# KIT-MBS/pydca

Hardware: AMD Instinct MI355X
Metric: plmDCA L-BFGS iterations/s (L=500 N=50000 q=21) (higher is better)
Workload: dtype f32

## Files before the change

### include/dca_hip.h

```cpp
#ifndef DCA_HIP_H
#define DCA_HIP_H

#include <stdbool.h>
#include <stddef.h>
#include <stdint.h>

#ifdef __cplusplus
extern "C" {
#endif

#define DCA_OK 0
#define DCA_ERR_ARG (-1)
#define DCA_ERR_IO (-2)
#define DCA_ERR_RESIDUE (-3)
#define DCA_ERR_NOMEM (-4)
#define DCA_ERR_HIP (-5)
#define DCA_ERR_NO_DEVICE (-6)
#define DCA_ERR_NOT_SPD (-7)
#define DCA_ERR_STATE (-8)

#define DCA_BIOMOLECULE_PROTEIN 1
#define DCA_BIOMOLECULE_RNA 2

#define DCA_F32 32
// ... 80 lines not shown
typedef int (*dca_comm_hook)(void* user, int op, void* buf_dev, size_t count, int dtype);
int dca_plm_set_vector_sharding(dca_ctx* ctx, int rank, int world, dca_comm_hook hook, void* user);

typedef struct {
    int status;
    int iterations;
    int evaluations;
    int finished;
    double fx, xnorm, gnorm, step;
    double seconds;
} dca_plm_stats;

int dca_plm_lbfgs_begin(dca_ctx* ctx, int max_iterations, int verbose);
int dca_plm_lbfgs_iterate(dca_ctx* ctx, int iterations, dca_plm_stats* stats_out);
int dca_plm_lbfgs_end(dca_ctx* ctx);

typedef struct dca_plm_args {
    int biomolecule;
    const char* msa_file;
    const uint8_t* msa;
    int num_seqs, seqs_len;
    float seqid, lambda_h, lambda_J;
    int max_iterations;
    int precision;
    const int* devices;
    int num_devices;
    int exchange_scheme;
    const char* rccl_path;
    int verbose;
} dca_plm_args;
// ... 130 lines not shown
```

### pydca_amd/_lib.py

```python
import ctypes as C
import os
import subprocess

import numpy as np

_HERE = os.path.dirname(os.path.abspath(__file__))
LIB_PATH = os.environ.get("DCA_LIB_PATH") or os.path.join(_HERE, "lib", "libdca_hip.so")

DCA_OK = 0
DCA_ERR_ARG, DCA_ERR_IO, DCA_ERR_RESIDUE = -1, -2, -3
DCA_ERR_NOMEM, DCA_ERR_HIP, DCA_ERR_NO_DEVICE, DCA_ERR_NOT_SPD, DCA_ERR_STATE = -4, -5, -6, -7, -8
DCA_F32, DCA_F64 = 32, 64
DCA_BIOMOLECULE_PROTEIN, DCA_BIOMOLECULE_RNA = 1, 2
CARRY_EXACT, CARRY_CHUNKED, CARRY_SERIAL = 0, 1, 2
PROTEIN, RNA = 1, 2


class DcaBackendError(RuntimeError):
    def __init__(self, code, msg):
        super().__init__("libdca_hip error %d: %s" % (code, msg))
        self.code = code


class PlmStats(C.Structure):
    _fields_ = [("status", C.c_int), ("iterations", C.c_int), ("evaluations", C.c_int), ("finished", C.c_int),
                ("fx", C.c_double), ("xnorm", C.c_double), ("gnorm", C.c_double), ("step", C.c_double),
                ("seconds", C.c_double)]
# ... 80 lines not shown
        "dca_plm_num_params": (sz, [i, i]),
        "dca_plm_init_x": (i, [vp]),
        "dca_plm_set_x": (i, [vp, vp, i]),
        "dca_plm_get_x": (i, [vp, vp, i]),
        "dca_plm_release": (i, [vp]),
        "dca_plm_gradient": (i, [vp, C.POINTER(d)]),
        "dca_plm_get_g": (i, [vp, vp, i]),
        "dca_plm_set_reduce_hook": (i, [vp, REDUCE_HOOK, vp]),
        "dca_mf_set_reduce_hook": (i, [vp, REDUCE_HOOK, vp]),
        "dca_di_from_arrays": (i, [vp, vp, i, vp, i, i, vp, vp]),
        "dca_di_from_fields": (i, [vp, vp, i, vp, vp, i, i, vp]),
        "dca_plm_set_vector_sharding": (i, [vp, i, i, COMM_HOOK, vp]),
        "dca_plm_lbfgs_begin": (i, [vp, i, i]),
        "dca_plm_lbfgs_iterate": (i, [vp, i, C.POINTER(PlmStats)]),
        "dca_plm_lbfgs_end": (i, [vp]),
        "dca_mf_set_row_window": (i, [vp, i, i]),
        "dca_comm_allgather_host": (i, [vp, vp, i, vp]),
        "dca_plm_scores": (i, [vp, i, vp]),
        "dca_plm_di_scores": (i, [vp, vp, i, vp]),
        "dca_mf_di_scores": (i, [vp, i, vp]),
        "dca_plm_pair_couplings": (i, [vp, vp, i, i, vp]),
        "dca_mf_fields": (i, [vp, vp]),
        "dca_encode_sequences": (i, [C.c_char_p, vp, i, i, i, i, vp, C.POINTER(i)]),
        "dca_plm_energies": (i, [vp, vp, i, vp]),
        "dca_plm_mutation_scan": (i, [vp, vp, vp]),
        "dca_mf_energies": (i, [vp, vp, i, vp]),
        "dca_mf_mutation_scan": (i, [vp, vp, vp]),
        "dca_plm_pseudo_likelihood": (i, [vp, vp, i, vp, vp, vp]),
        "dca_mf_pseudo_likelihood": (i, [vp, vp, i, vp, vp, vp]),
        "dca_plm_sample": (i, [vp, i, i, C.c_uint64, C.c_uint64, C.c_uint64, d, vp, vp]),
# ... 52 lines not shown
    }
    for name, (res, args) in sig.items():
        f = getattr(L, name)
        f.restype = res
        f.argtypes = args
    _lib = L
    return L


EXPORTS = ["dca_weights_work", "dca_compute_weights_sharded", "dca_weights_partial_counts", "dca_set_weight_counts", "dca_comm_unique_id",
           "dca_comm_init", "dca_comm_destroy", "dca_comm_abort", "dca_comm_info", "dca_plm_set_native_comm", "dca_mf_set_native_comm",
           "dca_last_error", "dca_version", "dca_device_count", "dca_release_cached_memory", "dca_device_blocks_in_use", "dca_read_msa", "dca_count_msa_lines", "dca_read_msa_alloc", "dca_mf_set_row_window", "dca_comm_allgather_host", "dca_fasta_shape", "dca_read_fasta", "dca_read_fasta_alloc", "dca_host_free", "dca_create",
           "dca_destroy", "dca_set_msa", "dca_compute_weights", "dca_set_weights", "dca_get_weights",
           "dca_get_weight_counts", "dca_get_meff", "dca_plm_configure", "dca_plm_configure_strips", "dca_plm_num_params", "dca_plm_init_x",
           "dca_plm_set_x", "dca_plm_get_x", "dca_plm_release", "dca_plm_gradient", "dca_plm_get_g", "dca_plm_set_reduce_hook", "dca_mf_set_reduce_hook", "dca_di_from_arrays", "dca_di_from_fields", "dca_plm_set_vector_sharding",
           "dca_plm_lbfgs_begin", "dca_plm_lbfgs_iterate", "dca_plm_lbfgs_end", "dca_plm_scores", "dca_plm_di_scores",
           "dca_mf_di_scores", "dca_plm_pair_couplings", "dca_mf_fields", "dca_mf_pair_couplings",
           "dca_encode_sequences", "dca_plm_energies", "dca_plm_mutation_scan", "dca_mf_energies", "dca_mf_mutation_scan",
           "dca_plm_pseudo_likelihood", "dca_mf_pseudo_likelihood",
           "dca_plm_sample", "dca_mf_sample", "dca_philox4x32_10",
           "dca_ar_configure", "dca_ar_num_params", "dca_ar_init_x", "dca_ar_set_x", "dca_ar_get_x", "dca_ar_gradient", "dca_ar_get_g",
           "dca_ar_fit", "dca_ar_log_probabilities", "dca_ar_sample", "dca_ar_release",
           "dca_ar_epistasis", "dca_ar_epistatic_scores",
           "dca_plm_bm_begin", "dca_plm_bm_iterate", "dca_plm_bm_freqs", "dca_plm_bm_chains", "dca_plm_bm_end",
           "dca_plm_ais", "dca_mf_ais", "dca_ais_estimate",
           "dca_hamming_nearest", "dca_sequence_statistics", "dca_alignment_statistics",
           "dca_three_site_values", "dca_three_site_scan", "dca_pca_fit", "dca_pca_project",
           "dca_mf_single_site_freqs",
           "dca_mf_pair_site_freqs", "dca_mf_corr_mat", "dca_mf_couplings", "dca_mf_scores", "dca_mf_run",
           "dca_mf_corr_from_freqs", "dca_spd_inverse", "dca_sw_scores", "dca_sw_align", "dca_scores_order", "dca_set_profiling", "dca_set_profiling_only", "dca_get_kernel_time",
           "dca_reset_kernel_times", "dca_plm_run", "plmdcaBackend", "freeFieldsAndCouplings"]
# ... 378 lines not shown
                return 1
        self._mf_hook = REDUCE_HOOK(tramp) if pyfunc is not None else C.cast(None, REDUCE_HOOK)
        check(self._l.dca_mf_set_reduce_hook(self._h, self._mf_hook, None))

    def plm_lbfgs_begin(self, max_iterations, verbose=False):
        check(self._l.dca_plm_lbfgs_begin(self._h, int(max_iterations), int(bool(verbose))))

    def plm_lbfgs_end(self):
        check(self._l.dca_plm_lbfgs_end(self._h))

    def plm_lbfgs_iterate(self, iterations):
        st = PlmStats()
        check(self._l.dca_plm_lbfgs_iterate(self._h, int(iterations), C.byref(st)))
        return st

    def plm_scores(self, apc=True):
        out = np.zeros(self.L * (self.L - 1) // 2, dtype=np.float64)
        check(self._l.dca_plm_scores(self._h, int(bool(apc)), _ptr(out)))
        return out

    def plm_di_scores(self, reg_fi, apc=False):
        reg_fi = np.ascontiguousarray(reg_fi, dtype=np.float64)
        if reg_fi.shape != (self.L, self.q):
            raise ValueError("reg_fi must be L x q")
        out = np.zeros(self.L * (self.L - 1) // 2, dtype=np.float64)
        check(self._l.dca_plm_di_scores(self._h, _ptr(reg_fi), int(bool(apc)), _ptr(out)))
        return out

    def di_from_arrays(self, couplings, layout, reg_fi, L, q, want_fields=False, want_di=True):
        couplings = np.ascontiguousarray(couplings, dtype=np.float64)
# ... 392 lines not shown
```

### pydca_amd/csrc/capi.cpp

```cpp
#include <cstdlib>

#include "dca_internal.h"

static thread_local char g_err[1024] = "";

void dca_set_error(const char* fmt, ...)
{
    va_list ap;
    va_start(ap, fmt);
    vsnprintf(g_err, sizeof(g_err), fmt, ap);
    va_end(ap);
}

void dca_flush_clocks(dca_ctx* ctx)
{
    for (auto& kv : ctx->clocks) {
        for (auto& pr : kv.second.pending) {
            float ms = 0.f;
            hipEventSynchronize(pr.second);
            if (hipEventElapsedTime(&ms, pr.first, pr.second) == hipSuccess) kv.second.ms += ms;
            hipEventDestroy(pr.first);
            hipEventDestroy(pr.second);
        }
        kv.second.pending.clear();
// ... 460 lines not shown
    if (hook && ctx->plm->native_mode == 4) { dca_set_error("configured for column strips: no reduce hook"); return DCA_ERR_STATE; }
    ctx->plm->hook = hook;
    ctx->plm->hook_user = user;
    if (hook && ctx->plm->native_mode == 1) ctx->plm->native_mode = 0;
    return DCA_OK;
}
int dca_plm_lbfgs_begin(dca_ctx* ctx, int max_iterations, int verbose)
{
    CHECK_CTX(ctx);
    DCA_TRY(need_plm(ctx));
    dca_bm_free(ctx);
    return ctx->plm->lbfgs_begin(max_iterations, verbose);
}
int dca_plm_lbfgs_iterate(dca_ctx* ctx, int iterations, dca_plm_stats* st) { CHECK_CTX(ctx); DCA_TRY(need_plm(ctx)); return ctx->plm->lbfgs_iterate(iterations, st); }
int dca_plm_lbfgs_end(dca_ctx* ctx) { CHECK_CTX(ctx); if (ctx->plm) ctx->plm->lbfgs_end(); return DCA_OK; }
int dca_plm_scores(dca_ctx* ctx, int apc, double* out) { CHECK_CTX(ctx); DCA_TRY(need_plm(ctx)); return ctx->plm->scores(apc, out); }
int dca_plm_energies(dca_ctx* ctx, const uint8_t* X, int n, double* energies_out)
{
    CHECK_CTX(ctx);
    DCA_TRY(need_plm(ctx));
    if (n < 0 || (n > 0 && (!X || !energies_out))) return DCA_ERR_ARG;
    PottsSource ps;
    DCA_TRY(ctx->plm->potts_source(&ps, false));
    return dca_potts_energies(ctx, ps, X, n, energies_out);
}
int dca_plm_mutation_scan(dca_ctx* ctx, const uint8_t* wildtype, double* dE_out)
{
    CHECK_CTX(ctx);
    DCA_TRY(need_plm(ctx));
    if (!wildtype || !dE_out) return DCA_ERR_ARG;
// ... 417 lines not shown
```

### pydca_amd/csrc/dca_internal.h

```cpp
#pragma once
#include <hip/hip_runtime.h>

#include <atomic>
#include <cstdarg>
#include <cstdint>
#include <cstdio>
#include <cstring>
#include <map>
#include <string>
#include <vector>

#include "../../include/dca_hip.h"
#include "potts_source.h"

void dca_set_error(const char* fmt, ...);

#define HIP_TRY(expr)                                                                   \
    do {                                                                                \
        hipError_t _e = (expr);                                                         \
        if (_e != hipSuccess) {                                                         \
            dca_set_error("%s failed: %s (%s:%d)", #expr, hipGetErrorString(_e), __FILE__, __LINE__); \
            return DCA_ERR_HIP;                                                         \
        }                                                                               \
    } while (0)
// ... 141 lines not shown
int dca_comm_native_sum_u32(dca_ctx* ctx, uint32_t* buf, size_t count);

struct PlmEngineBase {
    virtual ~PlmEngineBase() {}
    virtual int configure(double lambda_h, double lambda_J, int carry_mode, int chunk, int warmup,
                          int halo, int add_reg) = 0;
    virtual int configure_strips(double lambda_h, double lambda_J, int carry_mode, int chunk, int warmup) = 0;
    virtual int init_x() = 0;
    virtual int set_x(const void* x, int dtype) = 0;
    virtual int get_x(void* x, int dtype) = 0;
    virtual int get_g(void* g, int dtype) = 0;
    virtual int gradient(double* fx_out) = 0;
    virtual int lbfgs_begin(int max_iterations, int verbose) = 0;
    virtual int lbfgs_iterate(int iterations, dca_plm_stats* st) = 0;
    virtual void lbfgs_end() = 0;
    virtual int scores(int apc, double* out) = 0;
    virtual int di_scores(const double* reg_fi, int apc, double* out) = 0;
    virtual int pair_couplings(const int* pairs, int npairs, int shift, double* out) = 0;
    virtual int potts_source(PottsSource* out, bool one_gpu_only) = 0;
    virtual int bm_source(void** dx) = 0;
    virtual int set_vector_sharding(int rank, int world, dca_comm_hook hook, void* user) = 0;
    dca_reduce_hook hook = nullptr;
    void* hook_user = nullptr;
    virtual void weights_changed() = 0;
    virtual int set_native_comm(int mode) = 0;
    virtual bool configured_for_comm() const = 0;
    int native_mode = 0;
};
PlmEngineBase* dca_make_plm_engine(dca_ctx* ctx);

// ... 111 lines not shown
```

### pydca_amd/csrc/lbfgs_kernels.h

```cpp
#pragma once

#include "dca_internal.h"
#include "plm_plan.h"
#include "vec_kernels.h"

namespace {

template <bool DD> struct DotAcc;
template <> struct DotAcc<false> {
    double hi = 0.0;
    static constexpr double lo = 0.0;
    __device__ __forceinline__ void add(double a, double b) { hi += a * b; }
    __device__ __forceinline__ void wave_reduce() { for (int off = 32; off > 0; off >>= 1) hi += __shfl_down(hi, off); }
};
template <> struct DotAcc<true> {
    double hi = 0.0, lo = 0.0;
    __device__ __forceinline__ void add(double a, double b) { dd_add(hi, lo, __dmul_rn(a, b)); }
    __device__ __forceinline__ void wave_reduce() { dd_wave_reduce(hi, lo); }
};
template <int NV>
__device__ __forceinline__ void dot_block_store(double (*red)[2 * NV], int nv, double* __restrict__ partials, unsigned grid = 0)
{
    __syncthreads();
    if ((int)threadIdx.x < nv) {
// ... 19 lines not shown
            s0.add(av, bv); s1.add(cv, cv); s2.add(av, av);
        },
        { const double av = a[i]; const double bv = b[i]; const double cv = c[i]; s0.add(av, bv); s1.add(cv, cv); s2.add(av, av); })
    s0.wave_reduce(); s1.wave_reduce(); s2.wave_reduce();
    if ((threadIdx.x & 63) == 0) {
        double* r = red[threadIdx.x >> 6];
        r[0] = s0.hi; r[1] = s0.lo; r[2] = s1.hi; r[3] = s1.lo; r[4] = s2.hi; r[5] = s2.lo;
    }
    dot_block_store<3>(red, 3, partials);
}
struct VecPtrs5 { const void* s[5]; const void* y[5]; };
struct DirCoefs { double g; double s[5]; double y[5]; };

struct LbfgsDev { double SY[5][5]; double YY[5][5]; double ys[5]; DirCoefs cf; };
constexpr int kSlotDginit = 30;

__global__ void lbfgs_two_loop_kernel(double* __restrict__ scal, LbfgsDev* __restrict__ st, int e, int endNext, int bound, double gg)
{
    if (threadIdx.x != 0 || blockIdx.x != 0) return;
    constexpr int M = 5;
    const double ys = scal[1], yy = scal[2];
    const double* G5 = scal + 3;
    double Sg[M], Yg[M], alpha[M];
    st->ys[e] = ys;
    for (int k2 = 0; k2 < M; ++k2) {
        Sg[k2] = G5[k2]; Yg[k2] = G5[5 + k2];
        st->SY[e][k2] = G5[10 + k2];
        st->SY[k2][e] = G5[15 + k2];
        st->YY[e][k2] = G5[20 + k2];
        st->YY[k2][e] = G5[20 + k2];
// ... 231 lines not shown
    for (int b = lo_ + threadIdx.x; b < hi_; b += blockDim.x) dd_add2(hi, lo, parts[2 * (size_t)b], parts[2 * (size_t)b + 1]);
    dd_block_reduce(hi, lo, redHi, redLo);
    if (threadIdx.x == 0) { out[2 * blockIdx.x] = hi; out[2 * blockIdx.x + 1] = lo; }
}
__global__ __launch_bounds__(1024)
void dd_sum_final_kernel(const double* __restrict__ A, int nA, const double* __restrict__ B, int nB, double* __restrict__ out)
{
    __shared__ double redHi[1024], redLo[1024];
    double hi = 0.0, lo = 0.0;
    for (int b = threadIdx.x; b < nA; b += blockDim.x) dd_add2(hi, lo, A[2 * (size_t)b], A[2 * (size_t)b + 1]);
    for (int b = threadIdx.x; b < nB; b += blockDim.x) dd_add2(hi, lo, B[2 * (size_t)b], B[2 * (size_t)b + 1]);
    dd_block_reduce(hi, lo, redHi, redLo);
    if (threadIdx.x == 0) out[0] = hi + lo;
}

template <typename T>
__global__ __launch_bounds__(kVecThreads)
void vec_dot3_fx_kernel(const T* __restrict__ a, const T* __restrict__ b, const T* __restrict__ c, size_t n, double* __restrict__ partials,
                        const double* __restrict__ fxParts, int nFxParts, double* __restrict__ fxChunks)
{
    if (blockIdx.x >= (unsigned)kVecBlocks) {
        __shared__ double redHi[256], redLo[256];
        const int blk = (int)blockIdx.x - kVecBlocks;
        const int chunk = (nFxParts + kSumStageBlocks - 1) / kSumStageBlocks;
        const int lo_ = blk * chunk, hi_ = min(nFxParts, lo_ + chunk);
        double hi = 0.0, lo = 0.0;
        for (int p = lo_ + threadIdx.x; p < hi_; p += blockDim.x) dd_add2(hi, lo, fxParts[2 * (size_t)p], fxParts[2 * (size_t)p + 1]);
        dd_block_reduce(hi, lo, redHi, redLo);
        if (threadIdx.x == 0) { fxChunks[2 * blk] = hi; fxChunks[2 * blk + 1] = lo; }
        return;
    }
    __shared__ double red[kVecThreads / 64][6];
    DotAcc<sizeof(T) == 8> s0, s1, s2;
    DCA_VEC_LOOP_G(n, a, kVecBlocks,
        const Pack<T> pa = ldp_at(a + head_, iv); const Pack<T> pb = ldp_at(b + head_, iv); const Pack<T> pc = ldp_at(c + head_, iv);
        _Pragma("unroll") for (int k = 0; k < VEC; ++k) {
            const double av = pa.v[k]; const double bv = pb.v[k]; const double cv = pc.v[k];
            s0.add(av, bv); s1.add(cv, cv); s2.add(av, av);
        },
        { const double av = a[i]; const double bv = b[i]; const double cv = c[i]; s0.add(av, bv); s1.add(cv, cv); s2.add(av, av); })
    s0.wave_reduce(); s1.wave_reduce(); s2.wave_reduce();
    if ((threadIdx.x & 63) == 0) {
        double* r = red[threadIdx.x >> 6];
        r[0] = s0.hi; r[1] = s0.lo; r[2] = s1.hi; r[3] = s1.lo; r[4] = s2.hi; r[5] = s2.lo;
    }
    dot_block_store<3>(red, 3, partials, kVecBlocks);
}
__global__ __launch_bounds__(1024)
void vec_final_fx_kernel(const double* __restrict__ partials, int nb, int nk, double* __restrict__ out,
                         const double* __restrict__ A, int nA, const double* __restrict__ B, int nB, double* __restrict__ fxOut)
{
    __shared__ double redHi[1024], redLo[1024];
    const int k = blockIdx.x;
    double hi = 0.0, lo = 0.0;
    if (k < nk) {
        constexpr int NT = 256;
        if ((int)threadIdx.x < NT) {
            for (int b = threadIdx.x; b < nb; b += NT) dd_add2(hi, lo, partials[2 * ((size_t)k * nb + b)], partials[2 * ((size_t)k * nb + b) + 1]);
            redHi[threadIdx.x] = hi;
            redLo[threadIdx.x] = lo;
        }
        __syncthreads();
        for (int st = NT / 2; st > 0; st >>= 1) {
            if ((int)threadIdx.x < st) dd_add2(redHi[threadIdx.x], redLo[threadIdx.x], redHi[threadIdx.x + st], redLo[threadIdx.x + st]);
            __syncthreads();
        }
        if (threadIdx.x == 0) out[k] = redHi[0] + redLo[0];
        return;
    }
    for (int b = threadIdx.x; b < nA; b += blockDim.x) dd_add2(hi, lo, A[2 * (size_t)b], A[2 * (size_t)b + 1]);
    for (int b = threadIdx.x; b < nB; b += blockDim.x) dd_add2(hi, lo, B[2 * (size_t)b], B[2 * (size_t)b + 1]);
    dd_block_reduce(hi, lo, redHi, redLo);
    if (threadIdx.x == 0) fxOut[0] = hi + lo;
}

}
```

### pydca_amd/csrc/plm_engine.hip

```cpp
#include <algorithm>
#include <chrono>
#include <cmath>

#include "dca_internal.h"
#include "more_thuente.h"
#include "vec_kernels.h"
#include "plm_plan.h"
#include "plm_stages.h"
#include "lbfgs_kernels.h"

namespace {

static_assert(kPlanXcds == kNumXcd, "the planner deals strips to this many XCDs");

#ifdef DCA_ROUND_ABLATE
__global__ void round_to_f32_kernel(double* __restrict__ p, size_t n)
{
    for (size_t i = blockIdx.x * (size_t)blockDim.x + threadIdx.x; i < n; i += (size_t)gridDim.x * blockDim.x) p[i] = (double)(float)p[i];
}
inline int round_stage_mask() { const char* e = getenv("DCA_ROUND_F32_STAGES"); return e ? atoi(e) : 0; }
#define DCA_ROUND_STAGE(bit, ptr, count)                                                                             \
    do {                                                                                                             \
        if constexpr (sizeof(T) == 8)                                                                                \
            if (round_stage_mask() & (bit))                                                                          \
// ... 40 lines not shown
    bool lbfgs_alloc = false;
    bool deferFx = false, fxPending = false;
    size_t vlo = 0, vn = 0, Ppad = 0;
    dca_comm_hook comm = nullptr;
    void* comm_user = nullptr;
    int comm_rank = 0, comm_world = 0;

    struct {
        bool begun = false, finished = false;
        int status = 0, k = 1, end = 0, iters = 0, evals = 0, max_iterations = 0, verbose = 0;
        double fx = 0, step = 0, xnorm = 0, gnorm = 0, seconds = 0;
        double last_step = 0;
        double dginit = 0;
        bool dginit_on_device = false;
        bool trial_ready = false;
    } o;

    explicit PlmEngine(dca_ctx* c) : ctx(c), N(c->N), L(c->L), q(c->q), Ls(c->Ls) {}

    template <typename U> int dalloc(U** p, size_t n)
    {
        HIP_TRY(dca_dev_malloc(reinterpret_cast<void**>(p), std::max<size_t>(n, 1) * sizeof(U)));
        return DCA_OK;
    }
    void freeall() { each_buffer([](auto*& p) { dca_dev_free(p); p = nullptr; }); }
    ~PlmEngine() override { freeall(); }

    void weights_changed() override { configured = false; o = decltype(o)(); }

    int configure(double lh, double lJ, int cmode, int chunk_, int warm_, int halo_, int add_reg_) override
// ... 30 lines not shown
        lbfgs_alloc = false;
        o = decltype(o)();

        DCA_TRY(dalloc(&dx, plan.P + kVecPad)); DCA_TRY(dalloc(&dg, plan.P + kVecPad));
        DCA_TRY(dalloc(&dWt, (size_t)plan.Wrows * plan.Cs));
        DCA_TRY(dalloc(&dSR, (size_t)N * plan.Cs));
        DCA_TRY(dalloc(&dR, (size_t)(N + kNC) * plan.Cs));
        HIP_TRY(hipMemsetAsync(dR, 0, (size_t)(N + kNC) * plan.Cs * sizeof(T), ctx->stream));
        DCA_TRY(dalloc(&dG, plan.num_slabs() * plan.slab_elems()));
        DCA_TRY(dalloc(&dw, N));
        DCA_TRY(dalloc(&dXL, (size_t)ceil_div(plan.gUnits, JT) * JT * plan.Npad));
        DCA_TRY(dalloc(&dXT2, (size_t)plan.gUnits * plan.NT));
        DCA_TRY(dalloc(&dPairs, npairs));
        DCA_TRY(dalloc(&dFxPart, 2 * (size_t)plan.nFxPart));
        DCA_TRY(dalloc(&dRegPart, 2 * (size_t)(plan.nRegPart + kSumStageBlocks)));
        DCA_TRY(dalloc(&dVecPart, 2 * 27 * kVecBlocks));
        HIP_TRY(hipMemsetAsync(dRegPart, 0, 2 * (size_t)(plan.nRegPart + kSumStageBlocks) * sizeof(double), ctx->stream));
        HIP_TRY(hipMemsetAsync(dFxPart, 0, 2 * (size_t)plan.nFxPart * sizeof(double), ctx->stream));
        if (sizeof(T) == 8) {
            DCA_TRY(dalloc(&dColPart, 2 * (size_t)kColSumRowBlocks * Lq));
            if (q == 5) DCA_TRY(dalloc(&dColChunk, 2 * (size_t)plan.numScanChunks * Lq));
            DCA_TRY(dalloc(&dColSum, (size_t)Lq));
        }
        if (strips) { DCA_TRY(dalloc(&dGrecv, plan.grecvOff[sWorld])); DCA_TRY(dalloc(&dXsend, plan.xsendOff[sWorld])); DCA_TRY(dalloc(&dXrecv, plan.xrecvOff[sWorld])); }

        HIP_TRY(hipMemsetAsync(dx, 0, (plan.P + kVecPad) * sizeof(T), ctx->stream));
        HIP_TRY(hipMemsetAsync(dg, 0, (plan.P + kVecPad) * sizeof(T), ctx->stream));
        vlo = 0; vn = plan.P; Ppad = plan.P;
        if (strips) {
            native_mode = 4;
            vlo = plan.oLo; vn = plan.oHi - plan.oLo;
// ... 426 lines not shown
    }

    int gradient(double* fx_out) override
    {
        o.trial_ready = false;
        DCA_TRY(evaluate_async());
        DCA_TRY(reduce_scalars(0, 1));
        DCA_TRY(gather_vector(dg));
        DCA_TRY(read_scalars(1));
        if (fx_out) *fx_out = ctx->hScal[0];
        return DCA_OK;
    }

    void v_neg(T* d, const T* g) { hipLaunchKernelGGL(vec_neg_kernel<T>, dim3(kVecBlocks), dim3(kVecThreads), 0, ctx->stream, d + vlo, g + vlo, vn); }
    void v_step(T* x, const T* xp, double stp, const T* d) { hipLaunchKernelGGL(vec_step_kernel<T>, dim3(kVecBlocks), dim3(kVecThreads), 0, ctx->stream, x + vlo, xp + vlo, (T)stp, d + vlo, vn); }
    int eval_scalars(double* fx, double* gd, double* xx, double* gg)
    {
        if (fxPending) {
            double* const fxChunks = dRegPart + 2 * (size_t)plan.nRegPart;
            hipLaunchKernelGGL(vec_dot3_fx_kernel<T>, dim3(kVecBlocks + kSumStageBlocks), dim3(kVecThreads), 0, ctx->stream, dg + vlo, dd + vlo, dx + vlo, vn, dVecPart,
                               dRegPart, plan.nRegPart, fxChunks);
            hipLaunchKernelGGL(vec_final_fx_kernel, dim3(3 + 1), dim3(1024), 0, ctx->stream, dVecPart, kVecBlocks, 3, ctx->dScal + 1,
                               fxChunks, kSumStageBlocks, dFxPart, plan.nFxPart, ctx->dScal);
            fxPending = false;
        } else {
            hipLaunchKernelGGL(vec_dot3_kernel<T>, dim3(kVecBlocks), dim3(kVecThreads), 0, ctx->stream, dg + vlo, dd + vlo, dx + vlo, vn, dVecPart);
            hipLaunchKernelGGL(vec_final_kernel, dim3(3), dim3(256), 0, ctx->stream, dVecPart, kVecBlocks, 3, ctx->dScal + 1);
        }
        DCA_TRY(reduce_scalars(0, 4));
        DCA_TRY(read_scalars(kSlotDginit + 1));
        *fx = ctx->hScal[0]; *gd = ctx->hScal[1]; *xx = ctx->hScal[2]; *gg = ctx->hScal[3];
        if (o.dginit_on_device) { o.dginit = ctx->hScal[kSlotDginit]; o.dginit_on_device = false; }
        return DCA_OK;
    }

    int lbfgs_begin(int max_iterations, int verbose) override
    {
        if (!configured) { dca_set_error("dca_plm_configure first"); return DCA_ERR_STATE; }
        if (!lbfgs_alloc) {
            DCA_TRY(dalloc(&dxp, plan.P + kVecPad)); DCA_TRY(dalloc(&dgp, plan.P + kVecPad)); DCA_TRY(dalloc(&dd, plan.P + kVecPad));
            for (int i = 0; i < 5; ++i) { DCA_TRY(dalloc(&dS[i], plan.P + kVecPad)); DCA_TRY(dalloc(&dY[i], plan.P + kVecPad)); }
            HIP_TRY(hipMemsetAsync(dxp, 0, (plan.P + kVecPad) * sizeof(T), ctx->stream));
            HIP_TRY(hipMemsetAsync(dgp, 0, (plan.P + kVecPad) * sizeof(T), ctx->stream));
            HIP_TRY(hipMemsetAsync(dd, 0, (plan.P + kVecPad) * sizeof(T), ctx->stream));
            lbfgs_alloc = true;
        }
// ... 24 lines not shown

    int line_search(double* stp, double* f, double* xx, double* gg, int* rc_hip)
    {
        const MtParams params{1e-4, 0.9, 1e-16, 1e-20, 1e20, 5};
        const bool deferred = o.dginit_on_device;
        bool first = true;
        const int ls = mt_line_search(params, stp, f, &o.dginit, deferred, [&](double t, double* ft, double* dgt) {
            const bool ready = o.trial_ready && first && t == 1.0 && fused_step_ok();
            o.trial_ready = false; first = false;
            if (!ready) {
                v_step(dx, dxp, t, dd);
                DCA_ROUND_STAGE(32, dx, plan.P);
            }
            DCA_TRY(publish_x());
            DCA_TRY(evaluate_async(true, ready));
            return eval_scalars(ft, dgt, xx, gg);
        }, rc_hip);
        if (deferred && ls == LB_INCREASEGRADIENT) o.evals -= 1;
        return ls;
    }

    void lbfgs_end() override { o = decltype(o)(); }
    bool fused_step_ok() const
    {
#ifdef DCA_ROUND_ABLATE
        if (round_stage_mask()) return false;
#endif
        return knobs.fuseStep != 0 && native_mode == 0 && !hook && !comm && !strips && !stripEmulate && vlo == 0 && vn == plan.P &&
               plan.cS0 == 0 && plan.cS1 == L;
    }
    template <int Q> void launch_fused_step(const VecPtrs5& ptrs)
    {
        const int numJC = ceil_div(L, fused_step_jc(Q)), pairBlocks = ceil_div(L, fused_step_ti(Q, (int)sizeof(T))) * numJC;
        const size_t lds = (size_t)fused_step_ti(Q, (int)sizeof(T)) * fused_step_jc(Q) * Q * Q * sizeof(T);
        hipLaunchKernelGGL((lbfgs_dir_trial_expand_kernel<T, Q>), dim3((unsigned)(ceil_div(pairBlocks, 64) * 64 + ceil_div(L * Q, kFusedStepThreads))), dim3(kFusedStepThreads), lds,
                           ctx->stream, dd, dxp, dWt, dx, dg, ptrs, &dLb->cf, L, plan.Cs, numJC, pairBlocks);
    }
// ... 18 lines not shown
            }
            o.xnorm = std::sqrt(xx); o.gnorm = std::sqrt(gg);
            o.iters = o.k;
            o.last_step = o.step;
            if (o.verbose) {
                fprintf(stderr, "Iteration %d:\n", o.k);
                fprintf(stderr, "fx = %f, xnorm = %f, gnorm = %f, step = %f\n\n", o.fx, o.xnorm, o.gnorm, o.step);
            }
            const double xn = std::max(o.xnorm, 1.0);
            if (o.gnorm / xn <= 1e-3) { o.status = 0; o.finished = true; break; }
            if (o.max_iterations != 0 && o.max_iterations < o.k + 1) { o.status = LB_MAXIMUMITERATION; o.finished = true; break; }

            const int e = o.end;
            VecPtrs5 ptrs;
            for (int i = 0; i < M; ++i) { ptrs.s[i] = dS[i] + vlo; ptrs.y[i] = dY[i] + vlo; }
            {
                ScopedKernelClock kc(ctx, "lbfgs_vec");
                auto gram = [&](auto slot) {
                    hipLaunchKernelGGL((vec_diff_gram_kernel<T, decltype(slot)::value>), dim3(kVecBlocks), dim3(kVecThreads), 0, ctx->stream, ptrs, dS[e] + vlo, dY[e] + vlo,
                                       dx + vlo, dxp + vlo, dg + vlo, dgp + vlo, vn, dVecPart);
                };
                switch (e) {
                case 0: gram(std::integral_constant<int, 0>()); break;
                case 1: gram(std::integral_constant<int, 1>()); break;
                case 2: gram(std::integral_constant<int, 2>()); break;
                case 3: gram(std::integral_constant<int, 3>()); break;
                default: gram(std::integral_constant<int, 4>()); break;
                }
                hipLaunchKernelGGL(vec_final_kernel, dim3(27), dim3(256), 0, ctx->stream, dVecPart, kVecBlocks, 27, ctx->dScal + 1);
            }
            DCA_TRY(reduce_scalars(1, 27));
// ... 78 lines not shown
```

### pydca_amd/csrc/plm_plan.h

```cpp
#pragma once

#include <algorithm>
#include <cstddef>
#include <cstdlib>
#include <vector>

#include "../../include/dca_hip.h"

namespace {

constexpr int kPlanXcds = 8;
constexpr int kPairQ = 25;
constexpr int kNC = 128;
constexpr int kRowBytes = 512;
constexpr int kScatWavesC = 16;
constexpr int kCanonBlock = 16384;
static_assert(kCanonBlock % kNC == 0, "canonical blocks are whole tiles");
constexpr int kColSumRowBlocks = 64;
constexpr int kSumStageBlocks = 64;
constexpr int kMaxStripRanks = 64;
constexpr size_t kVecPad = 256;

struct PlmShape {
    int N = 0, L = 0, q = 0;
// ... 3 lines not shown
    int carryMode = DCA_CARRY_CHUNKED;
    int stripWorld = 1, stripRank = 0;
    bool strips = false;
};

struct PlmKnobs {
    int scatterRem = -1;
    int scatterSplit = -1;
    int scatterCanon = -1;
    int scatterWaves = -1;
    int plmPairs = -1;
    int scatterMerge = -1;
    int foldMerge = -1;
    int fuseFx = -1;
    int fuseStep = -1;
    bool is_set(int v) const { return v != -1; }
    static PlmKnobs from_env()
    {
        PlmKnobs k;
        auto rd = [](const char* name, int& v) { if (const char* e = getenv(name)) { v = atoi(e); if (v == -1) v = -2; } };
        rd("DCA_SCATTER_REM", k.scatterRem); rd("DCA_SCATTER_SPLIT", k.scatterSplit); rd("DCA_SCATTER_CANON", k.scatterCanon);
        rd("DCA_SCATTER_WAVES", k.scatterWaves); rd("DCA_PLM_PAIRS", k.plmPairs); rd("DCA_SCATTER_MERGE", k.scatterMerge);
        rd("DCA_FOLD_MERGE", k.foldMerge); rd("DCA_PLM_FUSE_FX", k.fuseFx);
        rd("DCA_PLM_FUSE_STEP", k.fuseStep);
        return k;
    }
};

struct PlmKernelShapes {
    int logitsSeqPerWg[3];
    int logitsJT[3];
    static int slot(int q) { return q == 21 ? 1 : q == kPairQ ? 2 : 0; }
};

struct ScatterLaunch {
    unsigned gridX = 0, gridY = 1;
    int N = 0, L = 0, Cs = 0, halo = 0, numChunks = 0, NT = 0, ctBase = 0, numPairs = 0, splitX = 1, numJG = 0, chunksPerSplit = 0;
    size_t slabElems = 0;
    int blockChunks = 0;
// ... 209 lines not shown
```

Before: 61.60.

## Fuse line-search dot products with L-BFGS history diff and Gram pass

Measured after the change: 62.43, median of 3. Within noise of the previous version (+1.3%).

```diff
diff --git a/include/dca_hip.h b/include/dca_hip.h
--- a/include/dca_hip.h
+++ b/include/dca_hip.h
@@ -118,6 +118,8 @@
 int dca_plm_lbfgs_begin(dca_ctx* ctx, int max_iterations, int verbose);
 int dca_plm_lbfgs_iterate(dca_ctx* ctx, int iterations, dca_plm_stats* stats_out);
 int dca_plm_lbfgs_end(dca_ctx* ctx);
+#define DCA_PLM_LBFGS_STATE_SCALARS 97
+int dca_plm_lbfgs_state(dca_ctx* ctx, int k, void* s_out, void* y_out, int dtype, double* scalars_out);
 
 typedef struct dca_plm_args {
     int biomolecule;
diff --git a/pydca_amd/_lib.py b/pydca_amd/_lib.py
--- a/pydca_amd/_lib.py
+++ b/pydca_amd/_lib.py
@@ -11,6 +11,7 @@
 DCA_ERR_ARG, DCA_ERR_IO, DCA_ERR_RESIDUE = -1, -2, -3
 DCA_ERR_NOMEM, DCA_ERR_HIP, DCA_ERR_NO_DEVICE, DCA_ERR_NOT_SPD, DCA_ERR_STATE = -4, -5, -6, -7, -8
 DCA_F32, DCA_F64 = 32, 64
+LBFGS_STATE_SCALARS = 97
 DCA_BIOMOLECULE_PROTEIN, DCA_BIOMOLECULE_RNA = 1, 2
 CARRY_EXACT, CARRY_CHUNKED, CARRY_SERIAL = 0, 1, 2
 PROTEIN, RNA = 1, 2
@@ -121,6 +122,7 @@
         "dca_plm_lbfgs_begin": (i, [vp, i, i]),
         "dca_plm_lbfgs_iterate": (i, [vp, i, C.POINTER(PlmStats)]),
         "dca_plm_lbfgs_end": (i, [vp]),
+        "dca_plm_lbfgs_state": (i, [vp, i, vp, vp, i, vp]),
         "dca_mf_set_row_window": (i, [vp, i, i]),
         "dca_comm_allgather_host": (i, [vp, vp, i, vp]),
         "dca_plm_scores": (i, [vp, i, vp]),
@@ -203,7 +205,7 @@
            "dca_destroy", "dca_set_msa", "dca_compute_weights", "dca_set_weights", "dca_get_weights",
            "dca_get_weight_counts", "dca_get_meff", "dca_plm_configure", "dca_plm_configure_strips", "dca_plm_num_params", "dca_plm_init_x",
            "dca_plm_set_x", "dca_plm_get_x", "dca_plm_release", "dca_plm_gradient", "dca_plm_get_g", "dca_plm_set_reduce_hook", "dca_mf_set_reduce_hook", "dca_di_from_arrays", "dca_di_from_fields", "dca_plm_set_vector_sharding",
-           "dca_plm_lbfgs_begin", "dca_plm_lbfgs_iterate", "dca_plm_lbfgs_end", "dca_plm_scores", "dca_plm_di_scores",
+           "dca_plm_lbfgs_begin", "dca_plm_lbfgs_iterate", "dca_plm_lbfgs_end", "dca_plm_lbfgs_state", "dca_plm_scores", "dca_plm_di_scores",
            "dca_mf_di_scores", "dca_plm_pair_couplings", "dca_mf_fields", "dca_mf_pair_couplings",
            "dca_encode_sequences", "dca_plm_energies", "dca_plm_mutation_scan", "dca_mf_energies", "dca_mf_mutation_scan",
            "dca_plm_pseudo_likelihood", "dca_mf_pseudo_likelihood",
@@ -612,6 +614,16 @@
         check(self._l.dca_plm_lbfgs_iterate(self._h, int(iterations), C.byref(st)))
         return st
 
+    def plm_lbfgs_state(self, dtype=np.float32):
+        P = int(self._l.dca_plm_num_params(self.L, self.q))
+        S = np.empty((5, P), dtype=dtype)
+        Y = np.empty((5, P), dtype=dtype)
+        scal = np.empty(LBFGS_STATE_SCALARS, dtype=np.float64)
+        dt = DCA_F32 if S.dtype == np.float32 else DCA_F64
+        for k in range(5):
+            check(self._l.dca_plm_lbfgs_state(self._h, k, _ptr(S[k]), _ptr(Y[k]), dt, _ptr(scal) if k == 0 else None))
+        return S, Y, scal
+
     def plm_scores(self, apc=True):
         out = np.zeros(self.L * (self.L - 1) // 2, dtype=np.float64)
         check(self._l.dca_plm_scores(self._h, int(bool(apc)), _ptr(out)))
diff --git a/pydca_amd/csrc/capi.cpp b/pydca_amd/csrc/capi.cpp
--- a/pydca_amd/csrc/capi.cpp
+++ b/pydca_amd/csrc/capi.cpp
@@ -498,6 +498,12 @@
 }
 int dca_plm_lbfgs_iterate(dca_ctx* ctx, int iterations, dca_plm_stats* st) { CHECK_CTX(ctx); DCA_TRY(need_plm(ctx)); return ctx->plm->lbfgs_iterate(iterations, st); }
 int dca_plm_lbfgs_end(dca_ctx* ctx) { CHECK_CTX(ctx); if (ctx->plm) ctx->plm->lbfgs_end(); return DCA_OK; }
+int dca_plm_lbfgs_state(dca_ctx* ctx, int k, void* s_out, void* y_out, int dtype, double* scalars_out)
+{
+    CHECK_CTX(ctx);
+    DCA_TRY(need_plm(ctx));
+    return ctx->plm->lbfgs_state(k, s_out, y_out, dtype, scalars_out);
+}
 int dca_plm_scores(dca_ctx* ctx, int apc, double* out) { CHECK_CTX(ctx); DCA_TRY(need_plm(ctx)); return ctx->plm->scores(apc, out); }
 int dca_plm_energies(dca_ctx* ctx, const uint8_t* X, int n, double* energies_out)
 {
diff --git a/pydca_amd/csrc/dca_internal.h b/pydca_amd/csrc/dca_internal.h
--- a/pydca_amd/csrc/dca_internal.h
+++ b/pydca_amd/csrc/dca_internal.h
@@ -179,6 +179,7 @@
     virtual int lbfgs_begin(int max_iterations, int verbose) = 0;
     virtual int lbfgs_iterate(int iterations, dca_plm_stats* st) = 0;
     virtual void lbfgs_end() = 0;
+    virtual int lbfgs_state(int k, void* s_out, void* y_out, int dtype, double* scalars_out) = 0;
     virtual int scores(int apc, double* out) = 0;
     virtual int di_scores(const double* reg_fi, int apc, double* out) = 0;
     virtual int pair_couplings(const int* pairs, int npairs, int shift, double* out) = 0;
diff --git a/pydca_amd/csrc/lbfgs_kernels.h b/pydca_amd/csrc/lbfgs_kernels.h
--- a/pydca_amd/csrc/lbfgs_kernels.h
+++ b/pydca_amd/csrc/lbfgs_kernels.h
@@ -57,6 +57,8 @@
 
 struct LbfgsDev { double SY[5][5]; double YY[5][5]; double ys[5]; DirCoefs cf; };
 constexpr int kSlotDginit = 30;
+constexpr int kSlotPostDots = 31;
+static_assert(28 + 1 + sizeof(LbfgsDev) / sizeof(double) + 2 == DCA_PLM_LBFGS_STATE_SCALARS, "dca_plm_lbfgs_state: dScal[0..27], dScal[kSlotDginit], LbfgsDev, two counts");
 
 __global__ void lbfgs_two_loop_kernel(double* __restrict__ scal, LbfgsDev* __restrict__ st, int e, int endNext, int bound, double gg)
 {
@@ -318,22 +320,23 @@
     if (threadIdx.x == 0) out[0] = hi + lo;
 }
 
+__device__ __forceinline__ void fx_chunk_block(const double* __restrict__ fxParts, int nFxParts, double* __restrict__ fxChunks)
+{
+    __shared__ double redHi[256], redLo[256];
+    const int blk = (int)blockIdx.x - kVecBlocks;
+    const int chunk = (nFxParts + kSumStageBlocks - 1) / kSumStageBlocks;
+    const int lo_ = blk * chunk, hi_ = min(nFxParts, lo_ + chunk);
+    double hi = 0.0, lo = 0.0;
+    for (int p = lo_ + threadIdx.x; p < hi_; p += blockDim.x) dd_add2(hi, lo, fxParts[2 * (size_t)p], fxParts[2 * (size_t)p + 1]);
+    dd_block_reduce(hi, lo, redHi, redLo);
+    if (threadIdx.x == 0) { fxChunks[2 * blk] = hi; fxChunks[2 * blk + 1] = lo; }
+}
 template <typename T>
 __global__ __launch_bounds__(kVecThreads)
 void vec_dot3_fx_kernel(const T* __restrict__ a, const T* __restrict__ b, const T* __restrict__ c, size_t n, double* __restrict__ partials,
                         const double* __restrict__ fxParts, int nFxParts, double* __restrict__ fxChunks)
 {
-    if (blockIdx.x >= (unsigned)kVecBlocks) {
-        __shared__ double redHi[256], redLo[256];
-        const int blk = (int)blockIdx.x - kVecBlocks;
-        const int chunk = (nFxParts + kSumStageBlocks - 1) / kSumStageBlocks;
-        const int lo_ = blk * chunk, hi_ = min(nFxParts, lo_ + chunk);
-        double hi = 0.0, lo = 0.0;
-        for (int p = lo_ + threadIdx.x; p < hi_; p += blockDim.x) dd_add2(hi, lo, fxParts[2 * (size_t)p], fxParts[2 * (size_t)p + 1]);
-        dd_block_reduce(hi, lo, redHi, redLo);
-        if (threadIdx.x == 0) { fxChunks[2 * blk] = hi; fxChunks[2 * blk + 1] = lo; }
-        return;
-    }
+    if (blockIdx.x >= (unsigned)kVecBlocks) { fx_chunk_block(fxParts, nFxParts, fxChunks); return; }
     __shared__ double red[kVecThreads / 64][6];
     DotAcc<sizeof(T) == 8> s0, s1, s2;
     DCA_VEC_LOOP_G(n, a, kVecBlocks,
@@ -350,9 +353,67 @@
     }
     dot_block_store<3>(red, 3, partials, kVecBlocks);
 }
+
+template <typename T, int E>
+__global__ __launch_bounds__(kVecThreads)
+void vec_dots_diff_gram_kernel(VecPtrs5 P, T* __restrict__ se, T* __restrict__ ye, const T* __restrict__ x, const T* __restrict__ xp,
+                               const T* __restrict__ g, const T* __restrict__ gp, const T* __restrict__ d, size_t n, double* __restrict__ partials,
+                               const double* __restrict__ fxParts, int nFxParts, double* __restrict__ fxChunks)
+{
+    if (blockIdx.x >= (unsigned)kVecBlocks) { fx_chunk_block(fxParts, nFxParts, fxChunks); return; }
+    __shared__ double red[kVecThreads / 64][60];
+    DotAcc<sizeof(T) == 8> dot[3];
+    DotAcc<sizeof(T) == 8> acc[27];
+    DCA_VEC_LOOP_G(n, se, kVecBlocks,
+        const Pack<T> px = ldp_at(x + head_, iv); const Pack<T> pxp = ldp_at(xp + head_, iv); const Pack<T> pg = ldp_at(g + head_, iv);
+        const Pack<T> pgp = ldp_at(gp + head_, iv); const Pack<T> pd = ldp_at(d + head_, iv);
+        Pack<T> psk[5]; Pack<T> pyk[5];
+        _Pragma("unroll") for (int k = 0; k < 5; ++k)
+            if (k != E) { psk[k] = ldp_at(static_cast<const T*>(P.s[k]) + head_, iv); pyk[k] = ldp_at(static_cast<const T*>(P.y[k]) + head_, iv); }
+        _Pragma("unroll") for (int u = 0; u < VEC; ++u) {
+            const double av = pg.v[u]; const double bv = pd.v[u]; const double cv = px.v[u];
+            dot[0].add(av, bv); dot[1].add(cv, cv); dot[2].add(av, av);
+        }
+        Pack<T> pse; Pack<T> pye;
+        _Pragma("unroll") for (int u = 0; u < VEC; ++u) {
+            pse.v[u] = px.v[u] - pxp.v[u]; pye.v[u] = pg.v[u] - pgp.v[u];
+            acc[0].add((double)pye.v[u], (double)pse.v[u]); acc[1].add((double)pye.v[u], (double)pye.v[u]);
+        }
+        psk[E] = pse; pyk[E] = pye;
+        stp_at(se + head_, iv, pse); stp_at(ye + head_, iv, pye);
+        _Pragma("unroll") for (int k = 0; k < 5; ++k) {
+            _Pragma("unroll") for (int u = 0; u < VEC; ++u) {
+                const double gv = pg.v[u]; const double sev = pse.v[u]; const double yev = pye.v[u];
+                const double sk = psk[k].v[u]; const double yk = pyk[k].v[u];
+                acc[2 + k].add(sk, gv); acc[7 + k].add(yk, gv); acc[12 + k].add(sev, yk); acc[17 + k].add(yev, sk); acc[22 + k].add(yev, yk);
+            }
+        },
+        { const double av = g[i]; const double bv = d[i]; const double cv = x[i];
+          dot[0].add(av, bv); dot[1].add(cv, cv); dot[2].add(av, av);
+          const T sev_ = x[i] - xp[i]; const T yev_ = g[i] - gp[i]; se[i] = sev_; ye[i] = yev_;
+          const double gv = g[i]; const double sev = sev_; const double yev = yev_;
+          acc[0].add(yev, sev); acc[1].add(yev, yev);
+          _Pragma("unroll") for (int k = 0; k < 5; ++k) {
+              const double sk = k == E ? sev : (double)static_cast<const T*>(P.s[k])[i]; const double yk = k == E ? yev : (double)static_cast<const T*>(P.y[k])[i];
+              acc[2 + k].add(sk, gv); acc[7 + k].add(yk, gv); acc[12 + k].add(sev, yk); acc[17 + k].add(yev, sk); acc[22 + k].add(yev, yk);
+          } })
+    const int lane = threadIdx.x & 63, wv = threadIdx.x >> 6;
+#pragma unroll
+    for (int v = 0; v < 3; ++v) {
+        dot[v].wave_reduce();
+        if (lane == 0) { red[wv][2 * v] = dot[v].hi; red[wv][2 * v + 1] = dot[v].lo; }
+    }
+#pragma unroll
+    for (int v = 0; v < 27; ++v) {
+        acc[v].wave_reduce();
+        if (lane == 0) { red[wv][6 + 2 * v] = acc[v].hi; red[wv][6 + 2 * v + 1] = acc[v].lo; }
+    }
+    dot_block_store<30>(red, 30, partials, kVecBlocks);
+}
 __global__ __launch_bounds__(1024)
 void vec_final_fx_kernel(const double* __restrict__ partials, int nb, int nk, double* __restrict__ out,
-                         const double* __restrict__ A, int nA, const double* __restrict__ B, int nB, double* __restrict__ fxOut)
+                         const double* __restrict__ A, int nA, const double* __restrict__ B, int nB, double* __restrict__ fxOut,
+                         int split, double* __restrict__ out2)
 {
     __shared__ double redHi[1024], redLo[1024];
     const int k = blockIdx.x;
@@ -369,7 +430,7 @@
             if ((int)threadIdx.x < st) dd_add2(redHi[threadIdx.x], redLo[threadIdx.x], redHi[threadIdx.x + st], redLo[threadIdx.x + st]);
             __syncthreads();
         }
-        if (threadIdx.x == 0) out[k] = redHi[0] + redLo[0];
+        if (threadIdx.x == 0) (k < split ? out + k : out2 + (k - split))[0] = redHi[0] + redLo[0];
         return;
     }
     for (int b = threadIdx.x; b < nA; b += blockDim.x) dd_add2(hi, lo, A[2 * (size_t)b], A[2 * (size_t)b + 1]);
diff --git a/pydca_amd/csrc/plm_engine.hip b/pydca_amd/csrc/plm_engine.hip
--- a/pydca_amd/csrc/plm_engine.hip
+++ b/pydca_amd/csrc/plm_engine.hip
@@ -78,6 +78,8 @@
         double dginit = 0;
         bool dginit_on_device = false;
         bool trial_ready = false;
+        bool post_done = false;
+        int post_passes = 0, post_accepted = 0;
     } o;
 
     explicit PlmEngine(dca_ctx* c) : ctx(c), N(c->N), L(c->L), q(c->q), Ls(c->Ls) {}
@@ -138,7 +140,7 @@
         DCA_TRY(dalloc(&dPairs, npairs));
         DCA_TRY(dalloc(&dFxPart, 2 * (size_t)plan.nFxPart));
         DCA_TRY(dalloc(&dRegPart, 2 * (size_t)(plan.nRegPart + kSumStageBlocks)));
-        DCA_TRY(dalloc(&dVecPart, 2 * 27 * kVecBlocks));
+        DCA_TRY(dalloc(&dVecPart, 2 * 30 * kVecBlocks));
         HIP_TRY(hipMemsetAsync(dRegPart, 0, 2 * (size_t)(plan.nRegPart + kSumStageBlocks) * sizeof(double), ctx->stream));
         HIP_TRY(hipMemsetAsync(dFxPart, 0, 2 * (size_t)plan.nFxPart * sizeof(double), ctx->stream));
         if (sizeof(T) == 8) {
@@ -595,22 +597,47 @@
 
     void v_neg(T* d, const T* g) { hipLaunchKernelGGL(vec_neg_kernel<T>, dim3(kVecBlocks), dim3(kVecThreads), 0, ctx->stream, d + vlo, g + vlo, vn); }
     void v_step(T* x, const T* xp, double stp, const T* d) { hipLaunchKernelGGL(vec_step_kernel<T>, dim3(kVecBlocks), dim3(kVecThreads), 0, ctx->stream, x + vlo, xp + vlo, (T)stp, d + vlo, vn); }
-    int eval_scalars(double* fx, double* gd, double* xx, double* gg)
-    {
-        if (fxPending) {
+    int eval_scalars(double* fx, double* gd, double* xx, double* gg, bool post = false)
+    {
+        o.post_done = false;
+        int dots = 1;
+        if (fxPending && post && knobs.fusePost != 0) {
+            const int e = o.end;
+            double* const fxChunks = dRegPart + 2 * (size_t)plan.nRegPart;
+            VecPtrs5 ptrs;
+            for (int i = 0; i < 5; ++i) { ptrs.s[i] = dS[i]; ptrs.y[i] = dY[i]; }
+            ScopedKernelClock kc(ctx, "lbfgs_vec");
+            auto pass = [&](auto slot) {
+                hipLaunchKernelGGL((vec_dots_diff_gram_kernel<T, decltype(slot)::value>), dim3(kVecBlocks + kSumStageBlocks), dim3(kVecThreads), 0, ctx->stream, ptrs,
+                                   dS[e], dY[e], dx, dxp, dg, dgp, dd, plan.P, dVecPart, dRegPart, plan.nRegPart, fxChunks);
+            };
+            switch (e) {
+            case 0: pass(std::integral_constant<int, 0>()); break;
+            case 1: pass(std::integral_constant<int, 1>()); break;
+            case 2: pass(std::integral_constant<int, 2>()); break;
+            case 3: pass(std::integral_constant<int, 3>()); break;
+            default: pass(std::integral_constant<int, 4>()); break;
+            }
+            hipLaunchKernelGGL(vec_final_fx_kernel, dim3(30 + 1), dim3(1024), 0, ctx->stream, dVecPart, kVecBlocks, 30, ctx->dScal + kSlotPostDots,
+                               fxChunks, kSumStageBlocks, dFxPart, plan.nFxPart, ctx->dScal, 3, ctx->dScal + 1);
+            fxPending = false;
+            o.post_done = true;
+            o.post_passes += 1;
+            dots = kSlotPostDots;
+        } else if (fxPending) {
             double* const fxChunks = dRegPart + 2 * (size_t)plan.nRegPart;
             hipLaunchKernelGGL(vec_dot3_fx_kernel<T>, dim3(kVecBlocks + kSumStageBlocks), dim3(kVecThreads), 0, ctx->stream, dg + vlo, dd + vlo, dx + vlo, vn, dVecPart,
                                dRegPart, plan.nRegPart, fxChunks);
             hipLaunchKernelGGL(vec_final_fx_kernel, dim3(3 + 1), dim3(1024), 0, ctx->stream, dVecPart, kVecBlocks, 3, ctx->dScal + 1,
-                               fxChunks, kSumStageBlocks, dFxPart, plan.nFxPart, ctx->dScal);
+                               fxChunks, kSumStageBlocks, dFxPart, plan.nFxPart, ctx->dScal, 3, nullptr);
             fxPending = false;
         } else {
             hipLaunchKernelGGL(vec_dot3_kernel<T>, dim3(kVecBlocks), dim3(kVecThreads), 0, ctx->stream, dg + vlo, dd + vlo, dx + vlo, vn, dVecPart);
             hipLaunchKernelGGL(vec_final_kernel, dim3(3), dim3(256), 0, ctx->stream, dVecPart, kVecBlocks, 3, ctx->dScal + 1);
         }
         DCA_TRY(reduce_scalars(0, 4));
-        DCA_TRY(read_scalars(kSlotDginit + 1));
-        *fx = ctx->hScal[0]; *gd = ctx->hScal[1]; *xx = ctx->hScal[2]; *gg = ctx->hScal[3];
+        DCA_TRY(read_scalars(kSlotPostDots + 3));
+        *fx = ctx->hScal[0]; *gd = ctx->hScal[dots]; *xx = ctx->hScal[dots + 1]; *gg = ctx->hScal[dots + 2];
         if (o.dginit_on_device) { o.dginit = ctx->hScal[kSlotDginit]; o.dginit_on_device = false; }
         return DCA_OK;
     }
@@ -665,13 +692,30 @@
             }
             DCA_TRY(publish_x());
             DCA_TRY(evaluate_async(true, ready));
-            return eval_scalars(ft, dgt, xx, gg);
+            return eval_scalars(ft, dgt, xx, gg, ready);
         }, rc_hip);
         if (deferred && ls == LB_INCREASEGRADIENT) o.evals -= 1;
         return ls;
     }
 
     void lbfgs_end() override { o = decltype(o)(); }
+    int lbfgs_state(int k, void* s_out, void* y_out, int dtype, double* scal_out) override
+    {
+        if (!configured || !lbfgs_alloc || !dLb) { dca_set_error("dca_plm_lbfgs_begin first"); return DCA_ERR_STATE; }
+        if (strips || comm || native_mode != 0) { dca_set_error("the L-BFGS state is read on one GPU with whole vectors"); return DCA_ERR_STATE; }
+        if ((s_out || y_out) && (k < 0 || k >= 5)) { dca_set_error("history slot out of range"); return DCA_ERR_ARG; }
+        if (dtype != DCA_F32 && dtype != DCA_F64) return DCA_ERR_ARG;
+        if (s_out) DCA_TRY(dtype == DCA_F32 ? download(dS[k], static_cast<float*>(s_out)) : download(dS[k], static_cast<double*>(s_out)));
+        if (y_out) DCA_TRY(dtype == DCA_F32 ? download(dY[k], static_cast<float*>(y_out)) : download(dY[k], static_cast<double*>(y_out)));
+        if (scal_out) {
+            HIP_TRY(hipStreamSynchronize(ctx->stream));
+            HIP_TRY(hipMemcpy(scal_out, ctx->dScal, 28 * sizeof(double), hipMemcpyDeviceToHost));
+            HIP_TRY(hipMemcpy(scal_out + 28, ctx->dScal + kSlotDginit, sizeof(double), hipMemcpyDeviceToHost));
+            HIP_TRY(hipMemcpy(scal_out + 29, dLb, sizeof(LbfgsDev), hipMemcpyDeviceToHost));
+            scal_out[95] = o.post_passes; scal_out[96] = o.post_accepted;
+        }
+        return DCA_OK;
+    }
     bool fused_step_ok() const
     {
 #ifdef DCA_ROUND_ABLATE
@@ -720,7 +764,10 @@
             const int e = o.end;
             VecPtrs5 ptrs;
             for (int i = 0; i < M; ++i) { ptrs.s[i] = dS[i] + vlo; ptrs.y[i] = dY[i] + vlo; }
-            {
+            if (o.post_done) {
+                o.post_done = false;
+                o.post_accepted += 1;
+            } else {
                 ScopedKernelClock kc(ctx, "lbfgs_vec");
                 auto gram = [&](auto slot) {
                     hipLaunchKernelGGL((vec_diff_gram_kernel<T, decltype(slot)::value>), dim3(kVecBlocks), dim3(kVecThreads), 0, ctx->stream, ptrs, dS[e] + vlo, dY[e] + vlo,
diff --git a/pydca_amd/csrc/plm_plan.h b/pydca_amd/csrc/plm_plan.h
--- a/pydca_amd/csrc/plm_plan.h
+++ b/pydca_amd/csrc/plm_plan.h
@@ -41,6 +41,7 @@
     int foldMerge = -1;
     int fuseFx = -1;
     int fuseStep = -1;
+    int fusePost = -1;
     bool is_set(int v) const { return v != -1; }
     static PlmKnobs from_env()
     {
@@ -49,7 +50,7 @@
         rd("DCA_SCATTER_REM", k.scatterRem); rd("DCA_SCATTER_SPLIT", k.scatterSplit); rd("DCA_SCATTER_CANON", k.scatterCanon);
         rd("DCA_SCATTER_WAVES", k.scatterWaves); rd("DCA_PLM_PAIRS", k.plmPairs); rd("DCA_SCATTER_MERGE", k.scatterMerge);
         rd("DCA_FOLD_MERGE", k.foldMerge); rd("DCA_PLM_FUSE_FX", k.fuseFx);
-        rd("DCA_PLM_FUSE_STEP", k.fuseStep);
+        rd("DCA_PLM_FUSE_STEP", k.fuseStep); rd("DCA_PLM_FUSE_POST", k.fusePost);
         return k;
     }
 };
```
